# mratsim/trace-of-radiance

Hardware: AMD Instinct MI355X
Metric: Msamples/s (pixels×spp/s) on book-1 random_scene (higher is better)
Workload: dtype f64

## Files before the change

### trace-of-radiance_amd/csrc/kernel/integrate_loop_plane.inc

```
            if constexpr (kWords) {
            const int x_first = h_xfirst;
            const int pl_first = h_plfirst;
            const bool mover = xkind >= 12;
            double f = 0.0;
            if (mover) {
              f = (time - SEG_T0) / SEG_DT;
              fc_f = f; fc_t0 = double_to_bits(SEG_T0); fc_dt = double_to_bits(SEG_DT);
            }
            const int i_begin = i;
            {
              const PlaneSeg ps = plane_seg(sray, pray, SEG_REACH, SEG_TRAVEL, f, h_rmax2);
              auto stage_one = [&](auto PWc) {
                constexpr int PW = decltype(PWc)::value;
                using Rec = std::conditional_t<PW == 2, float, double>;
                using RecPtr = std::conditional_t<PW == 2, cfptr, cdptr>;
                RecPtr rec = (RecPtr)(uintptr_t)(PW == 2 ? (const void*)p.xpl32 : (const void*)p.xpl) + ((long)pl_first + PW * (long)i);
                PlaneSeg32 ps32{};
                Rec n0, n1, n2 = 0, n3 = 0;
                if constexpr (PW == 2) {
                  ps32 = plane_seg32(sray, ps, h_r1, h_r2, (double)__int_as_float(__double2loint(h_r3)), (double)__int_as_float(__double2hiint(h_r3)));
                  n0 = __int_as_float(__double2loint(h_r0)); n1 = __int_as_float(__double2hiint(h_r0));
                } else {
                  n0 = h_r0; n1 = h_r1; n2 = h_r2; n3 = h_r3;
                }
                if (i != 0) {
                  n0 = rec[0]; n1 = rec[1];
                  if constexpr (PW == 4) { n2 = rec[2]; n3 = rec[3]; }
                }
                auto one = [&](unsigned m, int j) {
                  const Rec c0 = n0, c1 = n1, c2 = n2, c3 = n3;
                  n0 = rec[PW * (j + 1) + 0]; n1 = rec[PW * (j + 1) + 1];
                  if constexpr (PW == 4) {
                    n2 = rec[PW * (j + 1) + 2]; n3 = rec[PW * (j + 1) + 3];
                    return push_bit(m, plane_word_mov(ps, c0, c1, c2, c3));
                  } else {
                    (void)c2; (void)c3;
                    return push_bit(m, plane_word32(ps32, c0, c1));
                  }
                };
                int gb = seg_block0 + (int)((unsigned)i / (unsigned)kBlock);
                for (;;) {
                  while (i < seg_count && ((gb & 3) != 0 || seg_count - i < 4 * kBlock)) {
                    unsigned m = mw;
                    if (seg_real - i <= kBlock / 2) {
#pragma unroll
                      for (int j = 0; j < kBlock / 2; ++j) m = one(m, j);
                      m <<= (unsigned)(kBlock / 2);
                    } else {
#pragma unroll
                      for (int j = 0; j < kBlock; ++j) m = one(m, j);
                    }
                    rec += PW * kBlock;
                    mw = m;
                    gb_next = gb + 1;
                    i += kBlock;
                    if ((gb & 3) == 3) {
                      q[(unsigned)w_count * 64] = m;
                      nz = push_cond(nz, m != 0u);
                      w_count += 1;
                      if (w_count == kQCap) { full = true; break; }
                    }
                    gb += 1;
                  }
                  if (full || i >= seg_count) break;
                  int nw = (seg_count - i) / (4 * kBlock);
                  nw = nw < kQCap - w_count ? nw : kQCap - w_count;
                  unsigned m = 0;
                  int w = 0;
                  auto word = [&]() {
                    m = 0;
#pragma unroll
                    for (int j = 0; j < 4 * kBlock; ++j) m = one(m, j);
                    rec += PW * 4 * kBlock;
                    q[(unsigned)(w_count + w) * 64] = m;
                    nz = push_cond(nz, m != 0u);
                    w += 1;
                  };
#pragma unroll 1
                  while (w + 2 <= nw) { word(); word(); }
                  if (w < nw) word();
                  mw = m;
                  i += nw * 4 * kBlock;
                  gb += 4 * nw;
                  gb_next = gb;
                  w_count += nw;
                  if (w_count == kQCap) { full = true; break; }
                }
              };
              if (xkind == 13) stage_one(std::integral_constant<int, 4>{});
              else stage_one(std::integral_constant<int, 2>{});
            }
            {
              const int slot0 = seg_block0 * kBlock;
              const int slot_a = slot0 + i_begin, slot_b = slot0 + i;
              const int nb = gb_next & 3;
              const bool partial = !full && nb != 0;
              unsigned nzl = nz;
              if (partial) {
                const unsigned placed = mw << (unsigned)(8 * (4 - nb));
                q[(unsigned)w_count * 64] = placed;
                nzl = push_cond(nzl, placed != 0u);
              }
              const int k_a = (slot_a >> 5) - w_base, k_b = ((slot_b - 1) >> 5) - w_base;
              nzl &= (2u << (unsigned)(k_b - k_a)) - 1u;
              const bool shared_word = slot_b > slot_a && (slot_a & 31) != 0;
              unsigned sat_out = 0;
              if (shared_word) {
                const unsigned first_mask = 0xffffffffu >> (unsigned)(slot_a & 31);
                const unsigned w = q[(unsigned)k_a * 64];
                sat_out = w & ~first_mask;
                q[(unsigned)k_a * 64] = w & first_mask;
              }
              int k = k_a;
              unsigned cur = 0;
              unsigned* wp = q;
              const unsigned last_slot = (unsigned)(slot_b - 1);
              struct Pick { bool v; unsigned* w; int b; unsigned slot; };
              auto pick = [&]() {
                if (cur == 0 && nzl != 0) {
                  const int wb = 31 - __builtin_clz(nzl);
                  nzl &= ~(1u << wb);
                  k = k_b - wb;
                  wp = q + (unsigned)k * 64;
                  cur = *wp;
                }
                Pick c;
                c.v = cur != 0;
                c.b = 31 - __builtin_clz(cur | 1u);
                cur &= ~(1u << c.b);
                c.w = wp;
                const unsigned slot = ((unsigned)(w_base + k) << 5) + (unsigned)(31 - c.b);
                c.slot = slot < last_slot ? slot : last_slot;
                return c;
              };
              unsigned long long s2_t0 = 0;
              if (prof && lane == 0) s2_t0 = __builtin_readcyclecounter();
              if (slot_b > slot_a && xkind <= 12) {
                const ScreenSeg ss = screen2_seg(sray, SEG_REACH, SEG_TRAVEL, h_y, f);
                auto stage_two = [&](auto xr, auto KINDc) {
                  constexpr int KIND = decltype(KINDc)::value;
                  struct Cand { bool v; unsigned* w; int b; double r0, r1, r2, r3; };
                  constexpr bool kRecLds = std::is_same<decltype(xr), ldptr>::value;
                  unsigned lds_base = 0;
                  if constexpr (kRecLds) {
                    lds_base = (unsigned)(uintptr_t)xr;
                    asm volatile("" : "+v"(lds_base));
                  }
                  auto fetch = [&](Cand& c) {
                    const Pick pk = pick();
                    c.v = pk.v; c.w = pk.w; c.b = pk.b;
                    if constexpr (kRecLds) {
                      const ldptr r = (ldptr)(uintptr_t)(lds_base + pk.slot * 32u);
                      c.r0 = r[0]; c.r1 = r[1]; c.r2 = r[2]; c.r3 = r[3];
                    } else {
                      const auto r = xr + 4 * (long)pk.slot;
                      c.r0 = r[0]; c.r1 = r[1]; c.r2 = r[2]; c.r3 = r[3];
                    }
                  };
                  auto test = [&](const Cand& c) {
                    const int word = KIND == 12   ? screen2_movy_y<true>(ss, c.r0, c.r1, c.r2, c.r3)
                                     : KIND == 11 ? screen2_static_y<true>(ss, c.r0, c.r1, c.r2)
                                                  : screen2_static<true>(ss, c.r0, c.r1, c.r2, c.r3);
                    if (c.v && word >= 0) atomicAnd(c.w, ~(1u << c.b));
                  };
                  Cand ca{false, q, 0, 0.0, 0.0, 0.0, 0.0}, cb{false, q, 0, 0.0, 0.0, 0.0, 0.0};
                  fetch(ca);
                  for (;;) {
                    if (ballot64(ca.v || nzl != 0) == 0) break;
                    fetch(cb);
                    test(ca);
                    if (ballot64(cb.v || nzl != 0) == 0) break;
                    fetch(ca);
                    test(cb);
                  }
                };
                auto run = [&](auto KINDc) {
                  if (xstaged) stage_two((ldptr)stage + ((long)x_first - 4 * (long)slot0), KINDc);
                  else stage_two((gdptr)(uintptr_t)p.xrec + ((long)x_first - 4 * (long)slot0), KINDc);
                };
                if (xkind == 12) run(std::integral_constant<int, 12>{});
                else if (xkind == 11) run(std::integral_constant<int, 11>{});
                else run(std::integral_constant<int, 10>{});
                plane_ran = true;
              } else if (slot_b > slot_a) {
                double negmu, am;
                screen_margins(scr_s1 + SEG_REACH + SEG_TRAVEL * __builtin_fabs(f), scr_d1, a, negmu, am);
                const double neg_f = -f;
                auto stage_two = [&](auto xr) {
                  constexpr bool kRecLds = std::is_same<decltype(xr), ldptr>::value;
                  unsigned lds_base = 0;
                  if constexpr (kRecLds) {
                    lds_base = (unsigned)(uintptr_t)xr;
                    asm volatile("" : "+v"(lds_base));
                  }
                  for (;;) {
                    const Pick pk = pick();
                    if (ballot64(pk.v || nzl != 0) == 0) break;
                    double r0, r1, r2, r3, r4, r5, r6;
                    if constexpr (kRecLds) {
                      const ldptr r = (ldptr)(uintptr_t)(lds_base + pk.slot * 64u);
                      r0 = r[0]; r1 = r[1]; r2 = r[2]; r3 = r[3]; r4 = r[4]; r5 = r[5]; r6 = r[6];
                    } else {
                      const auto r = xr + 8 * (long)pk.slot;
                      r0 = r[0]; r1 = r[1]; r2 = r[2]; r3 = r[3]; r4 = r[4]; r5 = r[5]; r6 = r[6];
                    }
                    const int word = screen_filter(fma_(neg_f, r4, ox - r0), fma_(neg_f, r5, oy - r1), fma_(neg_f, r6, oz - r2), dx, dy, dz, a, negmu, am, r3);
                    if (pk.v && word >= 0) atomicAnd(pk.w, ~(1u << pk.b));
                  }
                };
                if (xstaged) stage_two((ldptr)stage + ((long)x_first - 8 * (long)slot0));
                else stage_two((gdptr)(uintptr_t)p.xrec + ((long)x_first - 8 * (long)slot0));
                plane_ran = true;
              }
              if (prof && lane == 0) prof_lds[kSecStage2] += __builtin_readcyclecounter() - s2_t0;
              if (shared_word) q[(unsigned)k_a * 64] |= sat_out;
              if (partial) mw = q[(unsigned)w_count * 64] >> (unsigned)(8 * (4 - nb));
            }
            }
```

### trace-of-radiance_amd/csrc/tor_scene.cpp

```cpp
#include "tor_scene.hpp"
#include "tor_knobs.hpp"

#include <algorithm>
#include <cmath>
#include <cstdlib>
#include <cstring>
#include <utility>

#include "tor_filter32.hpp"
#include "tor_kernels.hpp"
#include "tor_screen.hpp"

namespace tor {

namespace {

inline double i64_as_double(int64_t v) {
  double d;
  std::memcpy(&d, &v, 8);
  return d;
}

size_t padded(size_t c) { return (c + kPad - 1) / kPad * kPad; }

bool fill_material(double* c, const TorMaterial& m, int moving) {
  int64_t flags = (moving ? 1 : 0) | ((int64_t)m.kind << 8);
  c[13] = i64_as_double(flags);
  switch (m.kind) {
    case TOR_LAMBERTIAN:
      c[9] = m.u.lambertian.albedo.x; c[10] = m.u.lambertian.albedo.y; c[11] = m.u.lambertian.albedo.z;
      return true;
    case TOR_METAL:
      c[9] = m.u.metal.albedo.x; c[10] = m.u.metal.albedo.y; c[11] = m.u.metal.albedo.z;
      c[12] = m.u.metal.fuzz;
      return true;
    case TOR_DIELECTRIC: {
      const double ri = m.u.dielectric.refraction_index;
      c[12] = ri;
      const double inv = 1.0 / ri;
      double r0f = (1.0 - inv) / (1.0 + inv);
      double r0b = (1.0 - ri) / (1.0 + ri);
      c[9] = inv;
      c[10] = r0f * r0f;
      c[11] = r0b * r0b;
      return true;
    }
    default:
      return false;
  }
}

bool fill_cold(double* c, const TorHittableVariant& h, int64_t orig) {
  if (h.kind == TOR_SPHERE) {
    const TorSphere& s = h.u.sphere;
    c[0] = s.center.x; c[1] = s.center.y; c[2] = s.center.z;
    c[6] = 1.0 / s.radius;
    c[14] = i64_as_double(orig);
    c[15] = s.radius * s.radius;
    return fill_material(c, s.material, 0);
  }
  const TorMovingSphere& s = h.u.moving_sphere;
  c[0] = s.center0.x; c[1] = s.center0.y; c[2] = s.center0.z;
  c[3] = s.center1.x - s.center0.x; c[4] = s.center1.y - s.center0.y; c[5] = s.center1.z - s.center0.z;
  c[6] = 1.0 / s.radius;
  c[7] = s.time0; c[8] = s.time1 - s.time0;
  c[14] = i64_as_double(orig);
  c[15] = s.radius * s.radius;
  return fill_material(c, s.material, 1);
}

}

namespace {

struct TimeGroup {
  uint64_t k0, k1;
  std::vector<int64_t> ids;
};

void add_to_group(std::vector<TimeGroup>& groups, const TorMovingSphere& s, int64_t i) {
  uint64_t k0, k1;
  std::memcpy(&k0, &s.time0, 8);
  std::memcpy(&k1, &s.time1, 8);
  for (auto& g : groups)
    if (g.k0 == k0 && g.k1 == k1) {
      g.ids.push_back(i);
      return;
    }
  groups.push_back({k0, k1, {i}});
}

bool group_moves_along_y_only(const TorHittableVariant* objs, const TimeGroup& g) {
  for (int64_t idx : g.ids) {
    const TorMovingSphere& s = objs[idx].u.moving_sphere;
    if (!(s.center1.x - s.center0.x == 0.0 && s.center1.z - s.center0.z == 0.0)) return false;
  }
  return true;
}

double norm3(double x, double y, double z) { return std::sqrt(x * x + y * y + z * z); }

}

F32Options f32_options_for(const TorHittableVariant* objs, int64_t n) {
  F32Options o;
  std::vector<double> ax[3];
  for (int64_t i = 0; i < n; ++i) {
    const TorVec3* c = objs[i].kind == TOR_SPHERE ? &objs[i].u.sphere.center
                       : (objs[i].kind == TOR_MOVING_SPHERE ? &objs[i].u.moving_sphere.center0 : nullptr);
    if (!c || !std::isfinite(c->x) || !std::isfinite(c->y) || !std::isfinite(c->z)) continue;
    ax[0].push_back(c->x); ax[1].push_back(c->y); ax[2].push_back(c->z);
  }
  if (ax[0].empty()) return o;
  const size_t mid = ax[0].size() / 2;
  for (int a = 0; a < 3; ++a) {
    std::vector<double> t = ax[a];
    std::nth_element(t.begin(), t.begin() + mid, t.end());
    o.origin[a] = t[mid];
  }
  std::vector<double> dist(ax[0].size());
  for (size_t k = 0; k < dist.size(); ++k)
    dist[k] = norm3(ax[0][k] - o.origin[0], ax[1][k] - o.origin[1], ax[2][k] - o.origin[2]);
  std::nth_element(dist.begin(), dist.begin() + mid, dist.end());
  o.far_limit = 8.0 * dist[mid];
  if (!(o.far_limit > 0.0) || !std::isfinite(o.far_limit)) o.far_limit = 0.0;
  return o;
}

bool build_layout(const TorHittableVariant* objs, const std::vector<int64_t>& ids, HostLayout& out, std::string& err,
                  const F32Options* f32) {
  std::vector<int64_t> statics, statics32;
  std::vector<TimeGroup> groups, groups32;
  auto dist0 = [&](const TorVec3& c) {
    return norm3(c.x - f32->origin[0], c.y - f32->origin[1], c.z - f32->origin[2]);
  };
  for (int64_t i : ids) {
    const TorHittableVariant& h = objs[i];
    if (h.kind == TOR_SPHERE) {
      const TorSphere& s = h.u.sphere;
      const bool q = f32 && f32_eligible(dist0(s.center), 0.0, s.radius * s.radius) && dist0(s.center) <= f32->far_limit;
      (q ? statics32 : statics).push_back(i);
    } else if (h.kind == TOR_MOVING_SPHERE) {
      const TorMovingSphere& s = h.u.moving_sphere;
      const double dt = s.time1 - s.time0;
      const bool q = f32 && std::isfinite(s.time0) && std::isfinite(dt) && dt != 0.0 &&
                     f32_eligible(dist0(s.center0), norm3(s.center1.x - s.center0.x, s.center1.y - s.center0.y, s.center1.z - s.center0.z),
                                  s.radius * s.radius) &&
                     dist0(s.center0) <= f32->far_limit;
      add_to_group(q ? groups32 : groups, s, i);
    } else {
      err = "unknown HittableVariant kind";
      return false;
    }
  }
  struct Seg64 { int kind; std::vector<int64_t> ids; double t0, dt; int xkind; double y; };
  std::vector<Seg64> segs64;
  auto y_of = [&](int64_t i) { return objs[i].kind == TOR_SPHERE ? objs[i].u.sphere.center.y : objs[i].u.moving_sphere.center0.y; };
  auto r2_of = [&](int64_t i) {
    const double r = objs[i].kind == TOR_SPHERE ? objs[i].u.sphere.radius : objs[i].u.moving_sphere.radius;
    return r * r;
  };
  auto cut_by_y = [&](const std::vector<int64_t>& all_members, int kind, double t0, double dt, int xkind_rest, int xkind_uniform) {
    std::vector<int64_t> members, big;
    if (all_members.size() >= 2 * (size_t)kPad) {
      std::vector<double> r2s;
      for (int64_t i : all_members) r2s.push_back(r2_of(i));
      std::nth_element(r2s.begin(), r2s.begin() + r2s.size() / 2, r2s.end());
      const double limit = 16.0 * r2s[r2s.size() / 2];
      for (int64_t i : all_members) (r2_of(i) > limit ? big : members).push_back(i);
    } else {
      members = all_members;
    }
    const size_t big_at = segs64.size();
    if (!big.empty()) segs64.push_back({kind, big, t0, dt, xkind_rest, 0.0});
    if (members.empty()) return;
    std::vector<std::pair<uint64_t, std::vector<int64_t>>> by_y;
    for (int64_t i : members) {
      const double y = y_of(i);
      uint64_t b;
      std::memcpy(&b, &y, 8);
      bool found = false;
      for (auto& g : by_y)
        if (g.first == b) { g.second.push_back(i); found = true; break; }
      if (!found) by_y.push_back({b, {i}});
      if (by_y.size() > 64) break;
    }
    std::vector<int64_t> rest;
    std::vector<Seg64> uniform;
    if (by_y.size() <= 64 && xkind_uniform != 0) {
      for (auto& g : by_y)
        if (g.second.size() >= (size_t)kPad && std::isfinite(y_of(g.second[0]))) uniform.push_back({kind, g.second, t0, dt, xkind_uniform, y_of(g.second[0])});
      for (int64_t i : members) {
        const double y = y_of(i);
        bool in_uniform = false;
        for (const Seg64& u : uniform) {
          uint64_t a, b;
          std::memcpy(&a, &y, 8); std::memcpy(&b, &u.y, 8);
          if (a == b) { in_uniform = true; break; }
        }
        if (!in_uniform) rest.push_back(i);
      }
    } else {
      rest = members;
    }
    if (!rest.empty() && !big.empty() && rest.size() + big.size() < 48) {
      segs64[big_at].ids.insert(segs64[big_at].ids.end(), rest.begin(), rest.end());
      rest.clear();
    }
    if (!rest.empty()) segs64.push_back({kind, rest, t0, dt, xkind_rest, 0.0});
    for (Seg64& u : uniform) segs64.push_back(std::move(u));
  };
  if (!statics.empty()) cut_by_y(statics, 0, 0.0, 1.0, 10, 11);
  for (size_t gi = 0; gi < groups.size(); ++gi) {
    const TorMovingSphere& first = objs[groups[gi].ids[0]].u.moving_sphere;
    const double t0 = first.time0, dt = first.time1 - first.time0;
    const bool sane = std::isfinite(t0) && std::isfinite(dt) && dt != 0.0;
    TimeGroup gy{groups[gi].k0, groups[gi].k1, {}}, gg{groups[gi].k0, groups[gi].k1, {}};
    for (int64_t idx : groups[gi].ids) {
      const TorMovingSphere& s = objs[idx].u.moving_sphere;
      ((s.center1.x - s.center0.x == 0.0 && s.center1.z - s.center0.z == 0.0) ? gy : gg).ids.push_back(idx);
    }
    if (!gy.ids.empty()) cut_by_y(gy.ids, 1, t0, dt, sane ? 14 : 0, sane ? 12 : 0);
    if (!gg.ids.empty()) cut_by_y(gg.ids, 2, t0, dt, sane ? 13 : 0, 0);
  }
  for (size_t a = 0; a < segs64.size(); ++a) {
    if (!(segs64[a].kind == 0 && segs64[a].xkind == 11)) continue;
    for (size_t b = 0; b < segs64.size(); ++b) {
      Seg64& mv = segs64[b];
      if (!(mv.kind == 1 && mv.xkind == 12)) continue;
      uint64_t ya, yb;
      std::memcpy(&ya, &segs64[a].y, 8); std::memcpy(&yb, &mv.y, 8);
      if (ya != yb) continue;
      double ra = 0.0, rb = 0.0;
      for (int64_t i : segs64[a].ids) ra = std::fmax(ra, r2_of(i));
      for (int64_t i : mv.ids) rb = std::fmax(rb, r2_of(i));
      if (!(ra <= 4.0 * rb && rb <= 4.0 * ra)) continue;
      mv.ids.insert(mv.ids.end(), segs64[a].ids.begin(), segs64[a].ids.end());
      segs64.erase(segs64.begin() + (long)a);
      --a;
      break;
    }
  }
  std::stable_sort(segs64.begin(), segs64.end(), [](const Seg64& a, const Seg64& b) { return a.ids.size() > b.ids.size(); });
  auto as_mover = [&](int64_t idx) {
    if (objs[idx].kind == TOR_MOVING_SPHERE) return objs[idx].u.moving_sphere;
    TorMovingSphere m{};
    m.center0 = m.center1 = objs[idx].u.sphere.center;
    m.radius = objs[idx].u.sphere.radius;
    m.material = objs[idx].u.sphere.material;
    return m;
  };
  auto xs_of = [](int xkind) { return xkind == 0 ? 0 : (xkind >= 13 ? 8 : 4); };
  auto pw_of = [](int xkind) { return xkind == 0 ? 0 : (xkind == 13 ? 4 : 2); };
  auto slots_of = [&](const Seg64& sg, bool words) {
    size_t c = padded(sg.ids.size());
    if (words && sg.xkind >= 10 && sg.ids.size() >= 48 && c % 32 > 16) c = (c + 31) / 32 * 32;
    return c;
  };
  bool pad_words = true;
  {
    size_t t0 = 0, t1 = 0;
    for (const Seg64& sg : segs64) { t0 += slots_of(sg, false); t1 += slots_of(sg, true); }
    if ((t1 + 511) / 512 > (t0 + 511) / 512) pad_words = false;
  }
  size_t n_stat_p = 0, n_mov_p = 0, n_movy_p = 0, n_xrec = 0, n_xpl = 0;
  for (const Seg64& sg : segs64) {
    const size_t cp = slots_of(sg, pad_words);
    (sg.kind == 0 ? n_stat_p : (sg.kind == 1 ? n_movy_p : n_mov_p)) += cp;
    n_xrec += cp * (size_t)xs_of(sg.xkind);
    n_xpl += cp * (size_t)pw_of(sg.xkind);
  }
  std::vector<char> yonly32(groups32.size(), 0);
  size_t n32_slots = padded(statics32.size()), n32_floats = padded(statics32.size()) / 2 * 10;
  for (size_t gi = 0; gi < groups32.size(); ++gi) {
    const bool y = group_moves_along_y_only(objs, groups32[gi]);
    yonly32[gi] = y ? 1 : 0;
    n32_slots += padded(groups32[gi].ids.size());
    n32_floats += padded(groups32[gi].ids.size()) / 2 * (y ? 12 : 16);
  }
  out.n_sorted = n_stat_p + n_mov_p + n_movy_p + n32_slots;
  out.stat.assign(4 * n_stat_p + 8, 0.0);
  out.mov.assign(8 * n_mov_p + 8, 0.0);
  out.movy.assign(6 * n_movy_p + 8, 0.0);
  out.xrec.assign(n_xrec + 8, 0.0);
  out.xpl.assign(n_xpl + 8, 1e300);
  out.xpl32.assign(n_xpl + 16, kPlane32PadX);
  for (size_t k = 1; k < out.xpl32.size(); k += 2) out.xpl32[k] = kPlane32PadZ;
  out.xpl32seg.clear();
  out.hot32.assign(n32_floats + 32, 0.0f);
  out.cold.assign(16 * out.n_sorted + 16, 0.0);
  out.segs.clear();
  out.xsegs.clear();
  for (size_t k = 0; k < n_stat_p; ++k) out.stat[4 * k + 3] = -1.0;
  for (size_t k = 0; k < n_mov_p; ++k) out.mov[8 * k + 3] = -1.0;
  for (size_t k = 0; k < n_movy_p; ++k) out.movy[6 * k + 3] = -1.0;
  for (size_t k = 0; k < out.n_sorted; ++k) out.cold[16 * k + 15] = -1.0;

  auto up = [](double x) { return x * (1.0 + 0x1p-40); };
  size_t sorted = 0, stat_rec = 0, mov_rec = 0, movy_rec = 0, x_off = 0, pl_off = 0;
  for (const Seg64& sg : segs64) {
    const size_t cnt_p = slots_of(sg, pad_words);
    double reach = 0.0, travel = 0.0, rmax2 = 0.0;
    double xlo = INFINITY, xhi = -INFINITY, zlo = INFINITY, zhi = -INFINITY, dcx_max = 0.0, dcz_max = 0.0;
    auto grow = [&](double x, double z) {
      if (std::isfinite(x)) { xlo = std::fmin(xlo, x); xhi = std::fmax(xhi, x); }
      if (std::isfinite(z)) { zlo = std::fmin(zlo, z); zhi = std::fmax(zhi, z); }
    };
    for (int64_t idx : sg.ids) {
      if (sg.kind == 0) {
        const TorSphere& s = objs[idx].u.sphere;
        reach = std::fmax(reach, norm3(s.center.x, s.center.y, s.center.z) + std::fabs(s.radius));
        rmax2 = std::fmax(rmax2, s.radius * s.radius);
        grow(s.center.x, s.center.z);
      } else {
        const TorMovingSphere s = as_mover(idx);
        reach = std::fmax(reach, norm3(s.center0.x, s.center0.y, s.center0.z) + std::fabs(s.radius));
        rmax2 = std::fmax(rmax2, s.radius * s.radius);
        travel = std::fmax(travel, norm3(s.center1.x - s.center0.x, s.center1.y - s.center0.y, s.center1.z - s.center0.z));
        grow(s.center0.x, s.center0.z);
        dcx_max = std::fmax(dcx_max, std::fabs(s.center1.x - s.center0.x));
        dcz_max = std::fmax(dcz_max, std::fabs(s.center1.z - s.center0.z));
      }
    }
    const double ext_x = xhi >= xlo ? (xhi - xlo) + dcx_max : 0.0, ext_z = zhi >= zlo ? (zhi - zlo) + dcz_max : 0.0;
    const size_t first_rec = sg.kind == 0 ? stat_rec : (sg.kind == 1 ? movy_rec : mov_rec);
    out.segs.insert(out.segs.end(), {(double)sg.kind, (double)first_rec, (double)(cnt_p | ((cnt_p - sg.ids.size()) << 24)), (double)(sorted / kPad),
                                     sg.kind == 0 ? 0.0 : sg.t0, sg.kind == 0 ? 0.0 : sg.dt, up(reach), up(travel)});
    out.xsegs.insert(out.xsegs.end(), {(double)sg.xkind, (double)x_off, sg.y, (double)pl_off, rmax2, ext_x, ext_z, 0.0});
    double e32 = 0.0, cm32 = 0.0;
    const bool pl32 = sg.xkind >= 10 && sg.xkind != 13;
    const double orx = pl32 && xhi >= xlo ? 0.5 * xlo + 0.5 * xhi : 0.0, orz = pl32 && zhi >= zlo ? 0.5 * zlo + 0.5 * zhi : 0.0;
    for (size_t k = 0; k < sg.ids.size() && pl32; ++k) {
      const TorMovingSphere s = as_mover(sg.ids[k]);
      const float fx = plane32_offset(s.center0.x, orx, e32), fz = plane32_offset(s.center0.z, orz, e32);
      out.xpl32[pl_off + 2 * k] = fx; out.xpl32[pl_off + 2 * k + 1] = fz;
      cm32 = std::fmax(cm32, std::fmax(std::fabs((double)fx), std::fabs((double)fz)));
    }
    out.xpl32seg.insert(out.xpl32seg.end(), {orx, orz, e32, cm32});
    const size_t xs = (size_t)xs_of(sg.xkind), pw = (size_t)pw_of(sg.xkind);
    for (size_t k = 0; k < cnt_p && xs != 0; ++k) {
      double* x = &out.xrec[x_off + xs * k];
      if (xs == 4) x[sg.xkind == 10 ? 3 : 2] = 1e300;
      else x[3] = -1.0;
    }
    for (size_t k = 0; k < cnt_p && pw == 4; ++k) {
      double* pl = &out.xpl[pl_off + 4 * k];
      pl[2] = 0.0; pl[3] = 0.0;
    }
    for (size_t k = 0; k < sg.ids.size(); ++k) {
      const TorHittableVariant& hv = objs[sg.ids[k]];
      if (sg.kind == 0) {
        const TorSphere& s = hv.u.sphere;
        double* m = &out.stat[4 * (stat_rec + k)];
        m[0] = s.center.x; m[1] = s.center.y; m[2] = s.center.z;
        m[3] = s.radius * s.radius;
        double* x = &out.xrec[x_off + 4 * k];
        if (sg.xkind == 10) { x[0] = s.center.x; x[1] = s.center.y; x[2] = s.center.z; x[3] = screen2_K(s.center.x, s.center.y, s.center.z, s.radius * s.radius); }
        else { x[0] = s.center.x; x[1] = s.center.z; x[2] = screen2_Ky(s.center.x, s.center.z, s.radius * s.radius); x[3] = 0.0; }
        out.xpl[pl_off + 2 * k] = s.center.x; out.xpl[pl_off + 2 * k + 1] = s.center.z;
      } else {
        const TorMovingSphere s = as_mover(sg.ids[k]);
        const double dcx = s.center1.x - s.center0.x, dcy = s.center1.y - s.center0.y, dcz = s.center1.z - s.center0.z;
        if (sg.kind == 1) {
          double* m = &out.movy[6 * (movy_rec + k)];
          m[0] = s.center0.x; m[1] = s.center0.y; m[2] = s.center0.z;
          m[3] = s.radius * s.radius;
          m[4] = dcy;
          if (sg.xkind == 12) {
            double* x = &out.xrec[x_off + 4 * k];
            x[0] = s.center0.x; x[1] = s.center0.z; x[2] = screen2_Ky(s.center0.x, s.center0.z, s.radius * s.radius);
            x[3] = dcy;
          }
          if (sg.xkind != 0) { out.xpl[pl_off + 2 * k] = s.center0.x; out.xpl[pl_off + 2 * k + 1] = s.center0.z; }
        } else {
          double* m = &out.mov[8 * (mov_rec + k)];
          m[0] = s.center0.x; m[1] = s.center0.y; m[2] = s.center0.z;
          m[3] = s.radius * s.radius;
          m[4] = dcx; m[5] = dcy; m[6] = dcz;
          if (sg.xkind == 13) {
            double* pl = &out.xpl[pl_off + 4 * k];
            pl[0] = s.center0.x; pl[1] = s.center0.z; pl[2] = dcx; pl[3] = dcz;
          }
        }
        if (sg.xkind >= 13) {
          double* x = &out.xrec[x_off + 8 * k];
          x[0] = s.center0.x; x[1] = s.center0.y; x[2] = s.center0.z; x[3] = s.radius * s.radius;
          x[4] = dcx; x[5] = dcy; x[6] = dcz; x[7] = 0.0;
        }
      }
      if (!fill_cold(&out.cold[16 * (sorted + k)], hv, sg.ids[k])) { err = "unknown Material kind"; return false; }
    }
    (sg.kind == 0 ? stat_rec : (sg.kind == 1 ? movy_rec : mov_rec)) += cnt_p;
    x_off += cnt_p * xs;
    pl_off += cnt_p * pw;
    sorted += cnt_p;
  }

  size_t f_off = 0;
  auto emit32 = [&](const std::vector<int64_t>& members, int kind, double t0, double dt) -> bool {
    const int stride = kind == 5 ? 10 : (kind == 6 ? 12 : 16);
    const size_t cnt_p = padded(members.size());
    double mc0max = 0.0, dcmax = 0.0;
    for (size_t k = 0; k < cnt_p; ++k) {
      float* rec = &out.hot32[f_off + (k / 2) * (size_t)stride];
      const int h = (int)(k & 1);
      if (k >= members.size()) {
        rec[6 + h] = kF32PadR2;
        continue;
      }
      const TorHittableVariant& hv = objs[members[k]];
      const bool moving = hv.kind == TOR_MOVING_SPHERE;
      const TorVec3& c0 = moving ? hv.u.moving_sphere.center0 : hv.u.sphere.center;
      const double r = moving ? hv.u.moving_sphere.radius : hv.u.sphere.radius;
      const double q[3] = {c0.x - f32->origin[0], c0.y - f32->origin[1], c0.z - f32->origin[2]};
      const double mc0 = norm3(q[0], q[1], q[2]);
      rec[0 + h] = (float)q[0]; rec[2 + h] = (float)q[1]; rec[4 + h] = (float)q[2];
      rec[6 + h] = (float)(r * r);
      rec[8 + h] = f32_object_k(mc0, r * r, moving);
      mc0max = std::max(mc0max, mc0);
      if (moving) {
        const TorMovingSphere& s = hv.u.moving_sphere;
        const double dc[3] = {s.center1.x - s.center0.x, s.center1.y - s.center0.y, s.center1.z - s.center0.z};
        dcmax = std::max(dcmax, norm3(dc[0], dc[1], dc[2]));
        if (kind == 6) {
          rec[10 + h] = (float)dc[1];
        } else {
          rec[10 + h] = (float)dc[0]; rec[12 + h] = (float)dc[1]; rec[14 + h] = (float)dc[2];
        }
      }
      if (!fill_cold(&out.cold[16 * (sorted + k)], hv, members[k])) { err = "unknown Material kind"; return false; }
    }
    out.segs.insert(out.segs.end(), {(double)kind, (double)f_off, (double)cnt_p, (double)(sorted / kPad), t0, dt,
                                     (double)f32_round_up(mc0max * 1.000001), (double)f32_round_up(dcmax * 1.000001)});
    out.xsegs.insert(out.xsegs.end(), 8, 0.0);
    out.xpl32seg.insert(out.xpl32seg.end(), 4, 0.0);
    f_off += cnt_p / 2 * (size_t)stride;
    sorted += cnt_p;
    return true;
  };
  if (!statics32.empty() && !emit32(statics32, 5, 0.0, 1.0)) return false;
  for (size_t gi = 0; gi < groups32.size(); ++gi) {
    const TorMovingSphere& first = objs[groups32[gi].ids[0]].u.moving_sphere;
    if (!emit32(groups32[gi].ids, yonly32[gi] ? 6 : 7, first.time0, first.time1 - first.time0)) return false;
  }
  out.n_segs = (int)(out.segs.size() / 8);
  if (out.segs.empty()) out.segs.assign(8, 0.0);
  if (out.xsegs.empty()) out.xsegs.assign(8, 0.0);
  out.xhdr.assign(16 * (size_t)std::max(out.n_segs, 1) + 16, 0.0);
  for (int s = 0; s < out.n_segs; ++s) {
    const double* sg = &out.segs[8 * (size_t)s];
    const double* xs = &out.xsegs[8 * (size_t)s];
    double* h = &out.xhdr[16 * (size_t)s];
    int32_t gate = 0;
    const int n_real = ((int)sg[2] & 0xffffff) - ((int)sg[2] >> 24);
    if ((int)xs[0] >= 10 && n_real >= 48) {
      const double band = 2.0 * kPlaneGate * std::sqrt(xs[4]);
      const double e_min = std::fmin(xs[5], xs[6]), e_max = std::hypot(xs[5], xs[6]);
      gate = band < e_min ? 1 : (band < e_max ? 2 : 0);
    }
    const int32_t ints[8] = {(int32_t)xs[0], (int32_t)sg[0], (int32_t)sg[2], (int32_t)sg[3], (int32_t)sg[1], (int32_t)xs[1], (int32_t)xs[3], gate};
    std::memcpy(h, ints, sizeof(ints));
    h[4] = sg[4]; h[5] = sg[5]; h[6] = sg[6]; h[7] = sg[7];
    h[8] = xs[2]; h[9] = xs[4]; h[10] = xs[5]; h[11] = xs[6];
    const int xkind = (int)xs[0];
    if (xkind == 13) {
      for (size_t k = 0; k < 4; ++k) h[12 + k] = out.xpl[(size_t)xs[3] + k];
    } else if (xkind >= 10) {
      const double* o32 = &out.xpl32seg[4 * (size_t)s];
      std::memcpy(&h[12], &out.xpl32[(size_t)xs[3]], 8);
      h[13] = o32[0]; h[14] = o32[1];
      const float ec[2] = {o32[2] < 0x1p126 ? f32_up(o32[2]) : INFINITY, o32[3] < 0x1p126 ? f32_up(o32[3]) : INFINITY};
      std::memcpy(&h[15], ec, 8);
    }
  }
  const size_t n_trips = (out.n_sorted + 63) / 64;
  out.coop_trips.assign(4 * n_trips + 4, 0.0);
  for (size_t t = 0; t < n_trips; ++t) {
    bool any_mover = false, any_static = false, y_only = true, same_group = true, sane = true;
    uint64_t g0 = 0, g1 = 0;
    double t0 = 0.0, dt = 1.0;
    for (size_t k = 64 * t; k < 64 * (t + 1); ++k) {
      if (k >= out.n_sorted) { any_static = true; continue; }
      const double* cr = &out.cold[16 * k];
      int64_t flags;
      std::memcpy(&flags, &cr[13], 8);
      if (!(flags & 1)) { any_static = true; continue; }
      uint64_t b0, b1;
      std::memcpy(&b0, &cr[7], 8); std::memcpy(&b1, &cr[8], 8);
      if (!any_mover) { g0 = b0; g1 = b1; t0 = cr[7]; dt = cr[8]; }
      else if (b0 != g0 || b1 != g1) same_group = false;
      any_mover = true;
      if (!(cr[3] == 0.0 && cr[5] == 0.0)) y_only = false;
      if (!std::isfinite(cr[7]) || !std::isfinite(cr[8]) || cr[8] == 0.0) sane = false;
    }
    double kind = 3.0;
    if (!any_mover) kind = 0.0;
    else if (!any_static && same_group && sane) kind = y_only ? 1.0 : 2.0;
    out.coop_trips[4 * t + 0] = kind;
    out.coop_trips[4 * t + 1] = t0;
    out.coop_trips[4 * t + 2] = dt;
  }
  return true;
}

namespace {

constexpr size_t kTwoLevelMinBlocks = 96;

uint32_t spread10(uint32_t v) {
  v &= 0x3ff;
  v = (v | (v << 16)) & 0x030000FF;
  v = (v | (v << 8)) & 0x0300F00F;
  v = (v | (v << 4)) & 0x030C30C3;
  v = (v | (v << 2)) & 0x09249249;
  return v;
}

bool finite3(const TorVec3& v) { return std::isfinite(v.x) && std::isfinite(v.y) && std::isfinite(v.z); }

}

void build_accel(const TorHittableVariant* objs, int64_t n, HostAccel& out, const F32Options* f32) {
  out = HostAccel{};
  if (n < 64) return;
  std::vector<double> radii;
  radii.reserve((size_t)n);
  for (int64_t i = 0; i < n; ++i) {
    const double r = objs[i].kind == TOR_SPHERE ? objs[i].u.sphere.radius : objs[i].u.moving_sphere.radius;
    radii.push_back(std::fabs(r));
  }
  std::vector<double> tmp = radii;
  std::nth_element(tmp.begin(), tmp.begin() + tmp.size() / 2, tmp.end());
  const double median_r = tmp[tmp.size() / 2];
  std::vector<int64_t> always, spatial;
  for (int64_t i = 0; i < n; ++i) {
    bool ok = std::isfinite(radii[(size_t)i]) && radii[(size_t)i] <= 2.5 * median_r;
    if (objs[i].kind == TOR_SPHERE) {
      ok = ok && finite3(objs[i].u.sphere.center);
    } else if (objs[i].kind == TOR_MOVING_SPHERE) {
      const TorMovingSphere& s = objs[i].u.moving_sphere;
      const double dt = s.time1 - s.time0;
      ok = ok && finite3(s.center0) && finite3(s.center1) && std::isfinite(s.time0) && std::isfinite(dt) && dt != 0.0;
    } else {
      return;
    }
    (ok ? spatial : always).push_back(i);
  }
  if (spatial.size() < 32) return;
  std::string err;
  if (!build_layout(objs, always, out.always, err, f32)) return;
  std::vector<std::pair<uint32_t, int64_t>> keyed;
  keyed.reserve(spatial.size());
  const char* order_knob = knob("TOR_ACCEL_ORDER");
  const bool use_morton = order_knob && std::strcmp(order_knob, "morton") == 0;
  if (use_morton) {
    double lo[3] = {1e300, 1e300, 1e300}, hi[3] = {-1e300, -1e300, -1e300};
    auto c0 = [&](int64_t i, int a) {
      const TorVec3& c = objs[i].kind == TOR_SPHERE ? objs[i].u.sphere.center : objs[i].u.moving_sphere.center0;
      return a == 0 ? c.x : (a == 1 ? c.y : c.z);
    };
    for (int64_t i : spatial)
      for (int a = 0; a < 3; ++a) { lo[a] = std::min(lo[a], c0(i, a)); hi[a] = std::max(hi[a], c0(i, a)); }
    double ext = 1e-300;
    for (int a = 0; a < 3; ++a) ext = std::max(ext, hi[a] - lo[a]);
    for (int64_t i : spatial) {
      uint32_t q[3];
      for (int a = 0; a < 3; ++a) q[a] = (uint32_t)std::min(1023.0, std::max(0.0, (c0(i, a) - lo[a]) / ext * 1023.0));
      keyed.push_back({spread10(q[0]) | (spread10(q[2]) << 1) | (spread10(q[1]) << 2), i});
    }
    std::stable_sort(keyed.begin(), keyed.end());
  } else {
    const size_t ns = spatial.size();
    const bool second_level = ((ns + kPad - 1) / kPad + (size_t)kBoxFanout - 1) / (size_t)kBoxFanout > kTwoLevelMinBlocks;
    struct Hull { double lo[3], hi[3], mid[3]; };
    std::vector<Hull> hull(ns);
    for (size_t k = 0; k < ns; ++k) {
      const TorHittableVariant& ob = objs[spatial[k]];
      const bool mv = ob.kind == TOR_MOVING_SPHERE;
      const TorVec3& a0 = mv ? ob.u.moving_sphere.center0 : ob.u.sphere.center;
      const TorVec3& a1 = mv ? ob.u.moving_sphere.center1 : ob.u.sphere.center;
      const double r = radii[(size_t)spatial[k]];
      const double p0[3] = {a0.x, a0.y, a0.z}, p1[3] = {a1.x, a1.y, a1.z};
      for (int a = 0; a < 3; ++a) {
        hull[k].lo[a] = std::min(p0[a], p1[a]) - r;
        hull[k].hi[a] = std::max(p0[a], p1[a]) + r;
        hull[k].mid[a] = 0.5 * (p0[a] + p1[a]);
      }
    }
    std::vector<uint32_t> ord(ns), best_ord, cand;
// ... 268 lines not shown
```

### trace-of-radiance_amd/csrc/tor_screen.hpp

```cpp
#pragma once
#include "tor_math.hpp"

namespace tor {

#if defined(TOR_SCREEN_MUTATE) && TOR_SCREEN_MUTATE == 1
#define TOR_MARGIN(x) 0.0
#else
#define TOR_MARGIN(x) (x)
#endif
TOR_HD void screen_margins(double B, double d1, double a, double& negmu, double& am) {
  negmu = TOR_MARGIN(-(B * d1) * 0x1p-48);
  am = TOR_MARGIN(a * ((B * B) * 0x1p-45));
}
TOR_HD int screen_filter(double ocx, double ocy, double ocz, double dx, double dy, double dz, double a, double negmu,
                         double am, double r2) {
  const double hb = fma_(ocz, dz, fma_(ocy, dy, fma_(ocx, dx, negmu)));
  const double cc = fma_(ocz, ocz, fma_(ocy, ocy, fma_(ocx, ocx, -r2)));
  const double t = fma_(-a, cc, am);
  const double disc = fma_(hb, hb, t);
  const unsigned h = (unsigned)(double_to_bits(hb) >> 32), y = (unsigned)(double_to_bits(t) >> 32), z = (unsigned)(double_to_bits(disc) >> 32);
#if defined(__HIP_DEVICE_COMPILE__) && __has_builtin(__builtin_amdgcn_bitop3_b32)
  return (int)__builtin_amdgcn_bitop3_b32(h, y, z, 0x51);
#else
  return (int)((h | ~y) & ~z);
#endif
}

struct ScreenRay {
  double dnx, dny, dnz;
  double s1;
  double ox, oy, oz;
  bool wild;
};
struct ScreenSeg {
  double hx, hy, hz;
  double Pn;
  double a2x, a2y, a2z;
  double Tn;
  double ks;
  double fdy, gn, f2n;
};
TOR_HD ScreenRay screen2_ray(double ox, double oy, double oz, double dx, double dy, double dz, double a_strict) {
  ScreenRay r;
  const double inv = 1.0 / __builtin_sqrt(a_strict);
  r.dnx = dx * inv; r.dny = dy * inv; r.dnz = dz * inv;
  r.s1 = __builtin_fabs(ox) + __builtin_fabs(oy) + __builtin_fabs(oz);
  r.ox = ox; r.oy = oy; r.oz = oz;
  r.wild = !(a_strict >= 0x1p-900 && a_strict <= 0x1p900);
  return r;
}
TOR_HD double clamp01(double x) { return x > 0.0 ? (x < 1.0 ? x : 1.0) : 0.0; }
TOR_HD double fma_clamp_s(double a_uniform, double b, double c) {
#if defined(__HIP_DEVICE_COMPILE__)
  double r;
  asm("v_fma_f64 %0, %1, %2, %3 clamp" : "=v"(r) : "s"(a_uniform), "v"(b), "v"(c));
  return r;
#else
  return clamp01(fma_(a_uniform, b, c));
#endif
}
TOR_HD double fma_clamp_v(double a, double b, double c) {
#if defined(__HIP_DEVICE_COMPILE__)
  double r;
  asm("v_fma_f64 %0, %1, %2, %3 clamp" : "=v"(r) : "v"(a), "v"(b), "v"(c));
  return r;
#else
  return clamp01(fma_(a, b, c));
#endif
}
TOR_HD ScreenSeg screen2_seg(const ScreenRay& r, double reach, double travel, double y_rel, double f) {
  ScreenSeg s;
  const double B = r.s1 + reach + travel * __builtin_fabs(f);
  const double mu = TOR_MARGIN(B * 0x1p-47);
  const double M = TOR_MARGIN((B * B) * 0x1p-45);
  const bool wild = r.wild || !((B * B) * 0x1p-45 < __builtin_inf()) || !(f * f < __builtin_inf());
  uint64_t e = (double_to_bits(B) >> 52) & 0x7ffu;
  if (e < 3u) e = 3u;
  if (e > 0x7fbu) e = 0x7fbu;
  const double sg = bits_to_double((uint64_t)(0x7fcu - e) << 52), sg2 = sg * sg;
  const double oy = r.oy - y_rel;
  const double dnx = wild ? 0.0 : r.dnx, dny = wild ? 0.0 : r.dny, dnz = wild ? 0.0 : r.dnz;
  s.hx = sg * dnx; s.hy = sg * dny; s.hz = sg * dnz;
  const double P = fma_(oy, dny, fma_(r.oz, dnz, r.ox * dnx)) - mu;
  const double Q = fma_(oy, oy, fma_(r.oz, r.oz, r.ox * r.ox));
  s.Pn = wild ? 0.0 : -(sg * P);
  s.Tn = wild ? -__builtin_inf() : -(sg2 * (M - Q));
  const double n2 = wild ? 0.0 : -(sg2 + sg2);
  s.a2x = n2 * r.ox; s.a2y = n2 * oy; s.a2z = n2 * r.oz;
  s.ks = wild ? 0.0 : sg2;
  const double fw = wild ? 0.0 : f;
  s.fdy = fw * s.hy;
  s.gn = fw * s.a2y;
  s.f2n = sg2 * (fw * fw);
  return s;
}
TOR_HD int screen2_word(double nh, double tn) {
  const double q = fma_(-nh, nh, tn);
  return (int)(unsigned)(double_to_bits(q) >> 32);
}
template <bool kLane = false>
TOR_HD int screen2_static(const ScreenSeg& s, double cx, double cy, double cz, double K) {
  const double nh = kLane ? fma_clamp_v(cx, s.hx, fma_(cy, s.hy, fma_(cz, s.hz, s.Pn))) : fma_clamp_s(cx, s.hx, fma_(cy, s.hy, fma_(cz, s.hz, s.Pn)));
  const double tn = fma_(s.ks, K, fma_(s.a2x, cx, fma_(s.a2y, cy, fma_(s.a2z, cz, s.Tn))));
  return screen2_word(nh, tn);
}
template <bool kLane = false>
TOR_HD int screen2_static_y(const ScreenSeg& s, double cx, double cz, double K) {
  const double nh = kLane ? fma_clamp_v(cx, s.hx, fma_(cz, s.hz, s.Pn)) : fma_clamp_s(cx, s.hx, fma_(cz, s.hz, s.Pn));
  const double tn = fma_(s.ks, K, fma_(s.a2x, cx, fma_(s.a2z, cz, s.Tn)));
  return screen2_word(nh, tn);
}
template <bool kLane = false>
TOR_HD int screen2_movy_y(const ScreenSeg& s, double cx, double cz, double K, double dcy) {
  const double nh = kLane ? fma_clamp_v(dcy, s.fdy, fma_(cx, s.hx, fma_(cz, s.hz, s.Pn))) : fma_clamp_s(dcy, s.fdy, fma_(cx, s.hx, fma_(cz, s.hz, s.Pn)));
  const double w = fma_(s.f2n, dcy, s.gn);
  const double tn = fma_(s.ks, K, fma_(w, dcy, fma_(s.a2x, cx, fma_(s.a2z, cz, s.Tn))));
  return screen2_word(nh, tn);
}
TOR_HD double screen2_clampK(double k) { return __builtin_fmin(__builtin_fmax(k, -0x1.fffffffffffffp1023), 0x1.fffffffffffffp1023); }
TOR_HD double screen2_K(double cx, double cy, double cz, double r2) { return screen2_clampK(((cx * cx + cy * cy) + cz * cz) - r2); }
TOR_HD double screen2_Ky(double cx, double cz, double r2) { return screen2_clampK((cx * cx + cz * cz) - r2); }

struct PlaneRay {
  double nx, nz;
  double w2;
  bool all;
};
struct PlaneSeg {
  double nx, nz;
  double c0;
  double negthr;
  double fnx, fnz;
};
TOR_HD PlaneRay plane_ray(const ScreenRay& r) {
  PlaneRay pr;
  pr.nx = -r.dnz;
  pr.nz = r.dnx;
  pr.w2 = fma_(r.dnz, r.dnz, r.dnx * r.dnx);
  pr.all = r.wild || !(pr.w2 >= 0x1p-200);
  return pr;
}
TOR_HD PlaneSeg plane_seg(const ScreenRay& r, const PlaneRay& pr, double reach, double travel, double f, double rmax2) {
  PlaneSeg s;
  const double B = r.s1 + reach + travel * __builtin_fabs(f);
#if defined(TOR_SCREEN_MUTATE) && TOR_SCREEN_MUTATE <= 2
  const double M = 0.0;
  const double thr = rmax2 * pr.w2;
#else
  const double M = (B * B) * 0x1p-45;
  const double thr = (fma_(rmax2, 0x1p-40, rmax2) + M) * pr.w2;
#endif
  const bool all = pr.all || !(thr >= 0x1p-900 && thr < __builtin_inf());
  s.nx = all ? 0.0 : pr.nx;
  s.nz = all ? 0.0 : pr.nz;
  s.c0 = all ? 0.0 : -fma_(s.nx, r.ox, s.nz * r.oz);
  s.negthr = all ? -__builtin_inf() : -thr;
  s.fnx = all ? 0.0 : f * s.nx;
  s.fnz = all ? 0.0 : f * s.nz;
  return s;
}
TOR_HD int plane_word(const PlaneSeg& s, double cx, double cz) {
  const double v = fma_(s.nx, cx, fma_(s.nz, cz, s.c0));
  const double q = fma_(v, v, s.negthr);
  return (int)(unsigned)(double_to_bits(q) >> 32);
}
TOR_HD int plane_word_mov(const PlaneSeg& s, double c0x, double c0z, double dcx, double dcz) {
  const double v = fma_(s.nx, c0x, fma_(s.nz, c0z, fma_(s.fnx, dcx, fma_(s.fnz, dcz, s.c0))));
  const double q = fma_(v, v, s.negthr);
  return (int)(unsigned)(double_to_bits(q) >> 32);
}
constexpr float kPlane32PadX = 0x1p100f, kPlane32PadZ = 0x1.3c6ef3p99f;
constexpr double kPlane32Clamp = 0x1p100;
struct PlaneSeg32 {
  float nx, nz;
  float c0;
  float T;
};
TOR_HD float f32_up(double x) {
  float f = (float)x;
  if ((double)f < x) f = __builtin_bit_cast(float, __builtin_bit_cast(uint32_t, f) + 1u);
  return f;
}
TOR_HD PlaneSeg32 plane_seg32(const ScreenRay& r, const PlaneSeg& ps, double orx, double orz, double e32, double cm) {
  PlaneSeg32 s;
  const double ox = r.ox - orx, oz = r.oz - orz;
  const double co = __builtin_fabs(ox) + __builtin_fabs(oz);
  const double n1 = __builtin_fabs(ps.nx) + __builtin_fabs(ps.nz);
  const double thr = -ps.negthr;
  const float nx = (float)ps.nx, nz = (float)ps.nz;
  const double c0 = -fma_((double)nx, ox, (double)nz * oz);
#if defined(TOR_SCREEN_MUTATE) && TOR_SCREEN_MUTATE == 3
  (void)n1;
  const double T = __builtin_sqrt(thr);
  const float tf = (float)T;
#else
  const double T = (fma_(0x1p-20, __builtin_sqrt(thr) + n1 * e32, __builtin_sqrt(thr) + n1 * e32) +
                    fma_(n1, 0x1p-21, 0x1p-140) * ((cm + co) + e32) + 0x1p-140) * (1.0 + 0x1p-40);
  const float tf = T < 0x1p126 ? f32_up(T) : __builtin_inff();
#endif
  const bool all = !(ps.negthr > -__builtin_inf()) || !(cm <= 0x1p60 && co <= 0x1p60 && e32 <= 0x1p60) || !(tf < __builtin_inff());
  s.nx = all ? 0.0f : nx;
  s.nz = all ? 0.0f : nz;
  s.c0 = all ? 0.0f : (float)c0;
  s.T = all ? __builtin_inff() : tf;
  return s;
}
TOR_HD int plane_word32(const PlaneSeg32& s, float cx, float cz) {
  const float v = __builtin_fmaf(s.nx, cx, __builtin_fmaf(s.nz, cz, s.c0));
  const float q = __builtin_fabsf(v) - s.T;
  return (int)__builtin_bit_cast(uint32_t, q);
}
TOR_HD float plane32_offset(double c, double o, double& err_io) {
  const double d = c - o;
  const double bb = d - c, t = (c - (d - bb)) + (-o - bb);
  const double dc = __builtin_fmin(__builtin_fmax(d, -kPlane32Clamp), kPlane32Clamp);
  const float f = (float)dc;
  const double e = __builtin_fabs((d - (double)f) + t) * (1.0 + 0x1p-50);
  err_io = !(e < __builtin_inf()) ? __builtin_inf() : __builtin_fmax(err_io, e);
  return f;
}

constexpr double kPlaneGate = 16.0;
TOR_HD bool plane_pays(const PlaneRay& pr, double gate2, double rmax2, double sx, double sz) {
  const double e = fma_(__builtin_fabs(pr.nx), sx, __builtin_fabs(pr.nz) * sz);
  return !pr.all && (gate2 * rmax2) * pr.w2 < e * e;
}

}
```

Before: 3908.

## Software-pipeline scalar loads of fp32 plane records one group ahead in stage one

Result: faster. 4040 (median of 6 runs) (+3.4%).

```diff
diff --git a/trace-of-radiance_amd/csrc/kernel/integrate_loop_plane.inc b/trace-of-radiance_amd/csrc/kernel/integrate_loop_plane.inc
--- a/trace-of-radiance_amd/csrc/kernel/integrate_loop_plane.inc
+++ b/trace-of-radiance_amd/csrc/kernel/integrate_loop_plane.inc
@@ -67,6 +67,59 @@
                   nw = nw < kQCap - w_count ? nw : kQCap - w_count;
                   unsigned m = 0;
                   int w = 0;
+                  if constexpr (PW == 2 && kPlaneAhead == 1) {
+                    if (nw > 0) {
+                      typedef float __attribute__((ext_vector_type(16))) f16v;
+                      f16v ra, rb;
+#define TOR_FEED_REQ(nxt, off) asm volatile("s_load_dwordx16 %0, %3, %4" : "=&s"(nxt), "+v"(m), "+v"(mp) : "s"(rec), "i"(off))
+#define TOR_FEED_WAIT(cur) asm volatile("s_waitcnt lgkmcnt(0)" : "+s"(cur), "+v"(m), "+v"(mp))
+#define TOR_FEED_WAIT_REQ(cur, nxt, off) \
+  asm volatile("s_waitcnt lgkmcnt(0)\n\ts_load_dwordx16 %1, %4, %5" : "+s"(cur), "=&s"(nxt), "+v"(m), "+v"(mp) : "s"(rec), "i"(off))
+                      auto grp = [&](const f16v& b) {
+#pragma unroll
+                        for (int j = 0; j < kBlock; ++j) m = push_bit(m, plane_word32(ps32, b[2 * j], b[2 * j + 1]));
+                      };
+                      unsigned mp = 0;
+                      auto store = [&]() {
+                        q[(unsigned)(w_count + w) * 64] = mp;
+                        nz = push_cond(nz, mp != 0u);
+                        w += 1;
+                      };
+                      TOR_FEED_REQ(ra, 0);
+                      TOR_FEED_WAIT(ra);
+#pragma unroll 1
+                      while (w + 2 <= nw) {
+                        m = 0;
+                        TOR_FEED_REQ(rb, 64); grp(ra);
+                        TOR_FEED_WAIT_REQ(rb, ra, 128); grp(rb);
+                        TOR_FEED_WAIT_REQ(ra, rb, 192); grp(ra);
+                        TOR_FEED_WAIT_REQ(rb, ra, 256); grp(rb);
+                        mp = m;
+                        m = 0;
+                        TOR_FEED_WAIT_REQ(ra, rb, 320); store(); grp(ra);
+                        TOR_FEED_WAIT_REQ(rb, ra, 384); grp(rb);
+                        TOR_FEED_WAIT_REQ(ra, rb, 448); grp(ra);
+                        TOR_FEED_WAIT_REQ(rb, ra, 512); grp(rb);
+                        mp = m;
+                        TOR_FEED_WAIT(ra); store();
+                        rec += PW * 8 * kBlock;
+                      }
+                      if (w < nw) {
+                        m = 0;
+                        TOR_FEED_REQ(rb, 64); grp(ra);
+                        TOR_FEED_WAIT_REQ(rb, ra, 128); grp(rb);
+                        TOR_FEED_WAIT_REQ(ra, rb, 192); grp(ra);
+                        TOR_FEED_WAIT_REQ(rb, ra, 256); grp(rb);
+                        mp = m;
+                        TOR_FEED_WAIT(ra); store();
+                        rec += PW * 4 * kBlock;
+                      }
+#undef TOR_FEED_REQ
+#undef TOR_FEED_WAIT
+#undef TOR_FEED_WAIT_REQ
+                      n0 = ra[0]; n1 = ra[1];
+                    }
+                  } else {
                   auto word = [&]() {
                     m = 0;
 #pragma unroll
@@ -79,6 +132,7 @@
 #pragma unroll 1
                   while (w + 2 <= nw) { word(); word(); }
                   if (w < nw) word();
+                  }
                   mw = m;
                   i += nw * 4 * kBlock;
                   gb += 4 * nw;
diff --git a/trace-of-radiance_amd/csrc/tor_scene.cpp b/trace-of-radiance_amd/csrc/tor_scene.cpp
--- a/trace-of-radiance_amd/csrc/tor_scene.cpp
+++ b/trace-of-radiance_amd/csrc/tor_scene.cpp
@@ -284,7 +284,7 @@
   out.movy.assign(6 * n_movy_p + 8, 0.0);
   out.xrec.assign(n_xrec + 8, 0.0);
   out.xpl.assign(n_xpl + 8, 1e300);
-  out.xpl32.assign(n_xpl + 16, kPlane32PadX);
+  out.xpl32.assign(n_xpl + kPlaneSlackFloats, kPlane32PadX);
   for (size_t k = 1; k < out.xpl32.size(); k += 2) out.xpl32[k] = kPlane32PadZ;
   out.xpl32seg.clear();
   out.hot32.assign(n32_floats + 32, 0.0f);
diff --git a/trace-of-radiance_amd/csrc/tor_screen.hpp b/trace-of-radiance_amd/csrc/tor_screen.hpp
--- a/trace-of-radiance_amd/csrc/tor_screen.hpp
+++ b/trace-of-radiance_amd/csrc/tor_screen.hpp
@@ -169,6 +169,15 @@
   const double q = fma_(v, v, s.negthr);
   return (int)(unsigned)(double_to_bits(q) >> 32);
 }
+#ifdef TOR_PLANE_AHEAD
+constexpr int kPlaneAhead = TOR_PLANE_AHEAD;
+#else
+constexpr int kPlaneAhead = 1;
+#endif
+static_assert(kPlaneAhead == 0 || kPlaneAhead == 1, "two groups ahead would need scalar loads to return in order");
+constexpr int kPlaneGroupFloats = 16;
+constexpr int kPlaneSlackFloats = 16;
+static_assert(kPlaneSlackFloats >= kPlaneAhead * kPlaneGroupFloats && kPlaneSlackFloats >= 2, "the plane table's slack must cover stage one's read-ahead");
 constexpr float kPlane32PadX = 0x1p100f, kPlane32PadZ = 0x1.3c6ef3p99f;
 constexpr double kPlane32Clamp = 0x1p100;
 struct PlaneSeg32 {
```
